# ahuang73/HemoCell

Hardware: AMD Instinct MI355X
Metric: MLUPS + cell-vertex updates/s, 256^3 pipeflow 10% Hct (higher is better)
Workload: dtype f64

## Files before the change

hemocell_amd/csrc/ibm.hip:

```cpp
#include "cells.h"
#include <hipcub/hipcub.hpp>
#include <cstdlib>
#include <cstring>
#include <numeric>

namespace {

__global__ __launch_bounds__(256) void ibm_spread_kernel(LatView v, long n, const double *px, const double *py, const double *pz,
                                                         double *fx, double *fy, double *fz, const double *rx, const double *ry, const double *rz,
                                                         double *F, int limit_on, double f_limit, const int *vert_cell, const int *tag, const unsigned char *dead) {
  const long i = (long)blockIdx.x * 256 + threadIdx.x;
  if (i >= n) return;
  if (dead[i] || tag[vert_cell[i]] == 1) return;
  double f0 = fx[i], f1 = fy[i], f2 = fz[i];
  if (limit_on) {
    const double mag = sqrt((f0 * f0 + f1 * f1) + f2 * f2);
    if (mag > f_limit) {
      const double sc = f_limit / mag;
      f0 *= sc; f1 *= sc; f2 *= sc;
      fx[i] = f0; fy[i] = f1; fz[i] = f2;
    }
  }
  Stencil s;
  phi2_stencil(v, px[i], py[i], pz[i], s);
#pragma unroll
  for (int k = 0; k < 8; k++) {
    if (s.node[k] < 0) continue;
    v.dirty[s.node[k] >> 4] = v.epoch;
    unsafeAtomicAdd(&F[s.node[k]], ((rx ? rx[i] : 0.0) + f0) * s.w[k]);
    unsafeAtomicAdd(&F[v.npad + s.node[k]], ((ry ? ry[i] : 0.0) + f1) * s.w[k]);
    unsafeAtomicAdd(&F[2 * v.npad + s.node[k]], ((rz ? rz[i] : 0.0) + f2) * s.w[k]);
  }
}

__global__ __launch_bounds__(256) void spread_emit_kernel(LatView v, int nv, long n, const int *order, long ebase, const double *px, const double *py,
                                                          const double *pz, double *fx, double *fy, double *fz, const double *rx, const double *ry,
                                                          const double *rz, int limit_on, double f_limit, const int *tag, const unsigned char *dead,
                                                          unsigned int *keys, int *vals, double *c0, double *c1, double *c2) {
  const long g = (long)blockIdx.x * 256 + threadIdx.x;
  if (g >= n) return;
  const int cell = order[g / nv];
  const long i = (long)cell * nv + (g % nv);
  const long e0 = (ebase + g) * 8;
  const bool live = tag[cell] != 1 && !dead[i];
  Stencil s;
  double f0 = 0.0, f1 = 0.0, f2 = 0.0;
  if (live) {
    f0 = fx[i]; f1 = fy[i]; f2 = fz[i];
    if (limit_on) {
      const double mag = sqrt((f0 * f0 + f1 * f1) + f2 * f2);
      if (mag > f_limit) { const double sc = f_limit / mag; f0 *= sc; f1 *= sc; f2 *= sc; fx[i] = f0; fy[i] = f1; fz[i] = f2; }
    }
    if (rx) { f0 = rx[i] + f0; f1 = ry[i] + f1; f2 = rz[i] + f2; }
    phi2_stencil(v, px[i], py[i], pz[i], s);
  }
#pragma unroll
  for (int k = 0; k < 8; k++) {
    const bool adm = live && s.node[k] >= 0;
    keys[e0 + k] = adm ? (unsigned int)s.node[k] : 0xffffffffu;
    vals[e0 + k] = (int)(e0 + k);
    c0[e0 + k] = adm ? f0 * s.w[k] : 0.0; c1[e0 + k] = adm ? f1 * s.w[k] : 0.0; c2[e0 + k] = adm ? f2 * s.w[k] : 0.0;
  }
}

__global__ __launch_bounds__(256) void spread_gather_kernel(LatView v, long n, const unsigned int *keys, const int *vals, const double *c0, const double *c1,
                                                            const double *c2, double *F) {
  const long s = (long)blockIdx.x * 256 + threadIdx.x;
  if (s >= n) return;
  const unsigned int key = keys[s];
  if (key == 0xffffffffu || (s > 0 && keys[s - 1] == key)) return;
  double a0 = 0.0, a1 = 0.0, a2 = 0.0;
  for (long q = s; q < n && keys[q] == key; q++) { const int e = vals[q]; a0 += c0[e]; a1 += c1[e]; a2 += c2[e]; }
  v.dirty[key >> 4] = v.epoch;
  F[key] += a0; F[v.npad + key] += a1; F[2 * v.npad + key] += a2;
}

struct PopView {
  const double *f; const double *F; double bx, by, bz; long qs;
  hc::BodyRegions reg;
};

__device__ __forceinline__ void node_velocity(const LatView &v, const PopView &pv, int lx, int ly, int lz, long node, double u[3]) {
  if (v.halo_x && (lx <= -HALO || lx >= v.nx + HALO - 1)) { u[0] = u[1] = u[2] = 0.0; return; }
  if (v.halo_x && (lx == -1 || lx == v.nx)) {
    const double *hu = v.halo_u[lx < 0 ? 0 : 1];
    if (hu) { const long k = (long)ly * v.nz + lz; u[0] = hu[k]; u[1] = hu[v.ny_nz + k]; u[2] = hu[2L * v.ny_nz + k]; return; }
  }
  long xm = -(long)v.plane, xp = (long)v.plane;
  if (v.wrap_x) { if (lx == 0) xm = (long)(v.nx - 1) * v.plane; if (lx == v.nx - 1) xp = -(long)(v.nx - 1) * v.plane; }
  int ym = -v.nz, yp = v.nz, zm = -1, zp = 1; bool ymk = true, ypk = true, zmk = true, zpk = true;
  if (ly == 0) { if (v.per_y) ym = (v.ny - 1) * v.nz; else ymk = false; }
  if (ly == v.ny - 1) { if (v.per_y) yp = -(v.ny - 1) * v.nz; else ypk = false; }
  if (lz == 0) { if (v.per_z) zm = v.nz - 1; else zmk = false; }
  if (lz == v.nz - 1) { if (v.per_z) zp = -(v.nz - 1); else zpk = false; }
  double r = 0.0, jx = 0.0, jy = 0.0, jz = 0.0;
#define M(Q, CX, CY, CZ)                                                              \
  {                                                                                   \
    long off = 0; bool ok = true;                                                     \
    if (CX == 1) off += xm; else if (CX == -1) off += xp;                             \
    if (CY == 1) { off += ym; ok = ok && ymk; } else if (CY == -1) { off += yp; ok = ok && ypk; } \
    if (CZ == 1) { off += zm; ok = ok && zmk; } else if (CZ == -1) { off += zp; ok = ok && zpk; } \
    const double fq = ok ? pv.f[(long)Q * pv.qs + node + off] : 0.0;                 \
    r += fq;                                                                          \
    if (CX == 1) jx += fq; else if (CX == -1) jx += -fq;                              \
    if (CY == 1) jy += fq; else if (CY == -1) jy += -fq;                              \
    if (CZ == 1) jz += fq; else if (CZ == -1) jz += -fq;                              \
  }
  M(0, 0, 0, 0) M(1, -1, 0, 0) M(2, 0, -1, 0) M(3, 0, 0, -1) M(4, -1, -1, 0) M(5, -1, 1, 0)
  M(6, -1, 0, -1) M(7, -1, 0, 1) M(8, 0, -1, -1) M(9, 0, -1, 1) M(10, 1, 0, 0) M(11, 0, 1, 0)
  M(12, 0, 0, 1) M(13, 1, 1, 0) M(14, 1, -1, 0) M(15, 1, 0, 1) M(16, 1, 0, -1) M(17, 0, 1, 1)
  M(18, 0, 1, -1)
#undef M
  const double invRho = 1.0 / (1.0 + r);
  double bx = pv.bx, by = pv.by, bz = pv.bz;
  if (pv.reg.n) {
    int xg = v.x0 + lx;
    if (xg < 0) xg += v.nx_global; else if (xg >= v.nx_global) xg -= v.nx_global;
    region_force(pv.reg, xg, ly, lz, bx, by, bz);
  }
  u[0] = jx * invRho + (bx + pv.F[node]) / 2.0;
  u[1] = jy * invRho + (by + pv.F[v.npad + node]) / 2.0;
  u[2] = jz * invRho + (bz + pv.F[2 * v.npad + node]) / 2.0;
}

__global__ __launch_bounds__(256) void face_velocity_kernel(LatView v, PopView pv, int lx0, double *out0, int lx1, double *out1) {
  const int k = blockIdx.x * 256 + threadIdx.x;
  if (k >= v.ny_nz) return;
  const int lx = blockIdx.y ? lx1 : lx0;
  double *out = blockIdx.y ? out1 : out0;
  const int ly = k / v.nz, lz = k - ly * v.nz;
  const long node = (long)(lx + HALO) * v.plane + (long)ly * v.nz + lz;
  double u[3] = {0.0, 0.0, 0.0};
  if (v.mask[node] == 0) node_velocity(v, pv, lx, ly, lz, node, u);
  out[k] = u[0]; out[v.ny_nz + k] = u[1]; out[2L * v.ny_nz + k] = u[2];
}

__global__ __launch_bounds__(256) void ibm_interpolate_kernel(LatView v, PopView pv, long n, const double *px, const double *py,
                                                              const double *pz, double *vx, double *vy, double *vz, const int *vert_cell, const int *tag,
                                                              const unsigned char *dead) {
  const long i = (long)blockIdx.x * 256 + threadIdx.x;
  if (i >= n) return;
  if (dead[i] || tag[vert_cell[i]] == 1) return;
  Stencil s;
  phi2_stencil(v, px[i], py[i], pz[i], s);
  double a0 = 0.0, a1 = 0.0, a2 = 0.0;
#pragma unroll
  for (int k = 0; k < 8; k++) {
    if (s.node[k] < 0) continue;
    double u[3];
    node_velocity(v, pv, s.lx[k], s.ly[k], s.lz[k], s.node[k], u);
    a0 += (u[0] * s.w[k]); a1 += (u[1] * s.w[k]); a2 += (u[2] * s.w[k]);
  }
  vx[i] = a0; vy[i] = a1; vz[i] = a2;
}


constexpr int TILE_CAP = 5832;
constexpr int NODE_CAP = 1536;

struct Tile { int o[3]; int e[3]; int vol; int ow[3]; float r1, r2; };

__device__ __forceinline__ void tile_decode(const Tile &t, int i, int &tx, int &ty, int &tz) {
  const int q = (int)(((float)i + 0.5f) * t.r2);
  tz = i - q * t.e[2];
  tx = (int)(((float)q + 0.5f) * t.r1);
  ty = q - tx * t.e[1];
}

__device__ __forceinline__ int stencil_base(const LatView &v, double px, double py, double pz, int b[3]) {
  const double p[3] = {px, py, pz};
#pragma unroll
  for (int a = 0; a < 3; a++) { const long c = nearest_node(p[a]); b[a] = (int)c + ((p[a] < (double)c) ? -1 : 0); }
  return 0;
}

// ... 110 lines not shown
  }
  if (!inside) return false;
  if (nb[0] * nb[1] * nb[2] > 64) return false;
  if (threadIdx.x < 64) {
    const int l = threadIdx.x;
    bool near = false;
    if (l < nb[0] * nb[1] * nb[2]) {
      const int bz = l % nb[2], by = (l / nb[2]) % nb[1], bx = l / (nb[2] * nb[1]);
      near = v.wallbrick[((long)(b0[0] + bx) * v.nby + (b0[1] + by)) * v.nbz + (b0[2] + bz)] != 0;
    }
    const unsigned long long any = __ballot(near);
    if (l == 0) *s_near = any != 0ull;
  }
  __syncthreads();
  return *s_near == 0;
}

__device__ __forceinline__ bool cell_prologue(const LatView &v, int nv, long base, const double *px, const double *py, const double *pz,
                                              const unsigned char *dead, int *s_red, int *s_near, unsigned char *mt, Tile &t, VStencil vs[NVPT] PH_PARAM) {
  const int tid = threadIdx.x, nth = blockDim.x;
  double p[NVPT][3]; int b[NVPT][3]; bool live[NVPT];
  int lo[3] = {0x7fffffff, 0x7fffffff, 0x7fffffff}, hi[3] = {-0x7fffffff, -0x7fffffff, -0x7fffffff};
#pragma unroll
  for (int j = 0; j < NVPT; j++) {
    const int i = tid + j * nth;
    live[j] = i < nv && !(dead && dead[base + i]);
    if (live[j]) {
      p[j][0] = px[base + i]; p[j][1] = py[base + i]; p[j][2] = pz[base + i];
      stencil_base(v, p[j][0], p[j][1], p[j][2], b[j]);
#pragma unroll
      for (int a = 0; a < 3; a++) { lo[a] = min(lo[a], b[j][a]); hi[a] = max(hi[a], b[j][a] + 1); }
    }
  }
  block_bbox(lo, hi, s_red, t);
  STAMP(1);
  if (!tile_finish(v, t) || nv > NVPT * nth) return false;
  const bool clear = tile_is_clear(v, t, s_near);
  STAMP(2);
  if (!clear) {
#pragma unroll 4
    for (int i = tid; i < t.vol; i += nth) mt[i] = tile_mask(v, t, i);
    __syncthreads();
  }
  STAMP(3);
#pragma unroll
  for (int j = 0; j < NVPT; j++) {
    vs[j].adm = 0; vs[j].base = 0;
    if (live[j]) tile_stencil(t, clear ? nullptr : mt, p[j][0], p[j][1], p[j][2], b[j], vs[j]);
  }
  STAMP(4);
  return true;
}

__global__ __launch_bounds__(256) void ibm_spread_cell_kernel(LatView v, int nv, const double *px, const double *py, const double *pz,
                                                              double *fx, double *fy, double *fz, const double *rx, const double *ry, const double *rz,
                                                              double *F, int limit_on, double f_limit, int xcd_ranges, const int *tag, const unsigned char *vdead) {
  __shared__ double tile[TILE_CAP];
  __shared__ unsigned char mt[TILE_CAP];
  __shared__ int s_red[6 * MAXW], s_near;
  const int tid = threadIdx.x, nth = blockDim.x;
  PH_INIT
  const int cell = xcd_ranges ? xcd_contiguous((int)blockIdx.x, (int)gridDim.x) : (int)blockIdx.x;
  const int state = tag[cell];
  if (state == 1) return;
  STAMP(0);
  const unsigned char *dead = state == 2 ? vdead : nullptr;
  const long base = (long)cell * nv;
  const bool in_regs = nv <= NVPT * nth;
  double f[NVPT][3];
  if (in_regs) {
#pragma unroll
    for (int j = 0; j < NVPT; j++) {
      const int i = tid + j * nth;
      f[j][0] = f[j][1] = f[j][2] = 0.0;
      if (i < nv) { f[j][0] = fx[base + i]; f[j][1] = fy[base + i]; f[j][2] = fz[base + i]; }
    }
  }
  Tile t; VStencil vs[NVPT];
  bool tiled = cell_prologue(v, nv, base, px, py, pz, dead, s_red, &s_near, mt, t, vs PH_ARG);
  if (limit_on) {
    if (in_regs) {
#pragma unroll
      for (int j = 0; j < NVPT; j++) {
        const int i = tid + j * nth;
        if (i < nv) {
          const double mag = sqrt((f[j][0] * f[j][0] + f[j][1] * f[j][1]) + f[j][2] * f[j][2]);
          if (mag > f_limit) { const double sc = f_limit / mag; f[j][0] *= sc; f[j][1] *= sc; f[j][2] *= sc; fx[base + i] = f[j][0]; fy[base + i] = f[j][1]; fz[base + i] = f[j][2]; }
        }
      }
    } else {
      for (int i = tid; i < nv; i += nth) {
        const double f0 = fx[base + i], f1 = fy[base + i], f2 = fz[base + i];
        const double mag = sqrt((f0 * f0 + f1 * f1) + f2 * f2);
        if (mag > f_limit) { const double sc = f_limit / mag; fx[base + i] = f0 * sc; fy[base + i] = f1 * sc; fz[base + i] = f2 * sc; }
      }
    }
  }
  if (!tiled) {
    for (int i = tid; i < nv; i += nth) {
      if (dead && dead[base + i]) continue;
      Stencil s;
      phi2_stencil(v, px[base + i], py[base + i], pz[base + i], s);
      const double f0 = (rx ? rx[base + i] : 0.0) + fx[base + i], f1 = (ry ? ry[base + i] : 0.0) + fy[base + i], f2 = (rz ? rz[base + i] : 0.0) + fz[base + i];
#pragma unroll
      for (int k = 0; k < 8; k++) {
        if (s.node[k] < 0) continue;
        v.dirty[s.node[k] >> 4] = v.epoch;
        unsafeAtomicAdd(&F[s.node[k]], f0 * s.w[k]);
        unsafeAtomicAdd(&F[v.npad + s.node[k]], f1 * s.w[k]);
        unsafeAtomicAdd(&F[2 * v.npad + s.node[k]], f2 * s.w[k]);
      }
    }
    return;
  }
  const int sy = t.e[2], sx = t.e[1] * t.e[2];
  for (int i = tid; i < t.vol; i += nth) tile[i] = 0.0;
  __syncthreads();
  STAMP(5);
#pragma unroll
  for (int comp = 0; comp < 3; comp++) {
    const double *rc = comp == 0 ? rx : comp == 1 ? ry : rz;
    double *Fc = F + (long)comp * v.npad;
#pragma unroll
    for (int j = 0; j < NVPT; j++) {
      const int i = tid + j * nth;
      if (i >= nv || !vs[j].adm) continue;
      const double fv = (rc ? rc[base + i] : 0.0) + f[j][comp];
#pragma unroll
      for (int k = 0; k < 8; k++)
        if (vs[j].adm & (1u << k)) atomicAdd(&tile[vs[j].base + (k >> 2) * sx + ((k >> 1) & 1) * sy + (k & 1)], fv * vs[j].w[k]);
    }
    __syncthreads();
    STAMP(6 + 2 * comp);
    for (int i = tid; i < t.vol; i += nth) {
      const double val = tile[i];
      if (val != 0.0) {
        if (comp < 2) tile[i] = 0.0;
        int lx, ly, lz; const long node = tile_node(v, t, i, lx, ly, lz); v.dirty[node >> 4] = v.epoch;
        unsafeAtomicAdd(&Fc[node], val);
      }
    }
    if (comp < 2) __syncthreads();
    STAMP(7 + 2 * comp);
  }
}

__global__ __launch_bounds__(256) void ibm_interpolate_cell_kernel(LatView v, PopView pv, int nv, const double *px, const double *py,
                                                                   const double *pz, double *vx, double *vy, double *vz, const int *slots, int xcd_ranges,
                                                                   const int *tag, const unsigned char *vdead) {
  constexpr unsigned short FREE = 0xFFFF, MARK = 0xFFFE;
  __shared__ unsigned short slot[TILE_CAP];
  __shared__ __attribute__((aligned(16))) unsigned char raw[TILE_CAP > 2 * NODE_CAP ? TILE_CAP : 2 * NODE_CAP];
  unsigned char *mt = raw; unsigned short *list = reinterpret_cast<unsigned short *>(raw);
  __shared__ double ux[NODE_CAP], uy[NODE_CAP], uz[NODE_CAP];
  __shared__ int s_red[6 * MAXW], s_count, s_near;
  const int tid = threadIdx.x, nth = blockDim.x;
  const int cell = slots ? slots[blockIdx.x] : (xcd_ranges ? xcd_contiguous((int)blockIdx.x, (int)gridDim.x) : (int)blockIdx.x);
  const int state = tag[cell];
  if (state == 1) return;
  const unsigned char *dead = state == 2 ? vdead : nullptr;
  const long base = (long)cell * nv;
  Tile t; VStencil vs[NVPT];
  PH_INIT
  bool tiled = cell_prologue(v, nv, base, px, py, pz, dead, s_red, &s_near, mt, t, vs PH_ARG);
  const int sy = t.e[2], sx = t.e[1] * t.e[2];
  if (tiled) {
    for (int i = tid; i < t.vol; i += nth) slot[i] = FREE;
    if (tid == 0) s_count = 0;
    __syncthreads();
#pragma unroll
    for (int j = 0; j < NVPT; j++)
#pragma unroll
      for (int k = 0; k < 8; k++) if (vs[j].adm & (1u << k)) slot[vs[j].base + (k >> 2) * sx + ((k >> 1) & 1) * sy + (k & 1)] = MARK;
    __syncthreads();
    for (int i0 = 0; i0 < t.vol; i0 += nth) {
      const int i = i0 + tid;
      const bool marked = i < t.vol && slot[i] == MARK;
      const unsigned long long b = __ballot(marked);
      int first = 0;
      if ((tid & 63) == 0 && b) first = atomicAdd(&s_count, (int)__popcll(b));
      first = __shfl(first, 0);
      if (marked) {
        const int n = first + (int)__popcll(b & ((1ull << (tid & 63)) - 1ull));
        if (n < NODE_CAP) { slot[i] = (unsigned short)n; list[n] = (unsigned short)i; }
      }
    }
    __syncthreads();
    STAMP(12);
    if (s_count > NODE_CAP) tiled = false;
  }
  if (tiled) {
    const int n = s_count;
    for (int k = tid; k < n; k += nth) {
      int lx, ly, lz;
      const long node = tile_node(v, t, list[k], lx, ly, lz);
      double u[3];
      node_velocity(v, pv, lx, ly, lz, node, u);
      ux[k] = u[0]; uy[k] = u[1]; uz[k] = u[2];
    }
    __syncthreads();
    STAMP(13);
#pragma unroll
    for (int j = 0; j < NVPT; j++) {
      const int i = tid + j * nth;
      if (i >= nv) continue;
      double a0 = 0.0, a1 = 0.0, a2 = 0.0;
#pragma unroll
      for (int k = 0; k < 8; k++) {
        if (!(vs[j].adm & (1u << k))) continue;
        const int q = slot[vs[j].base + (k >> 2) * sx + ((k >> 1) & 1) * sy + (k & 1)];
        a0 += (ux[q] * vs[j].w[k]); a1 += (uy[q] * vs[j].w[k]); a2 += (uz[q] * vs[j].w[k]);
      }
      vx[base + i] = a0; vy[base + i] = a1; vz[base + i] = a2;
    }
    STAMP(14);
    return;
  }
  for (int i = tid; i < nv; i += nth) {
    if (dead && dead[base + i]) continue;
    Stencil s;
    phi2_stencil(v, px[base + i], py[base + i], pz[base + i], s);
    double a0 = 0.0, a1 = 0.0, a2 = 0.0;
#pragma unroll
    for (int k = 0; k < 8; k++) {
      if (s.node[k] < 0) continue;
      double u[3];
      node_velocity(v, pv, s.lx[k], s.ly[k], s.lz[k], s.node[k], u);
      a0 += (u[0] * s.w[k]); a1 += (u[1] * s.w[k]); a2 += (u[2] * s.w[k]);
    }
    vx[base + i] = a0; vy[base + i] = a1; vz[base + i] = a2;
  }
}

}

static int g_ibm_per_vertex = 0;
extern "C" int hc_debug_ibm_per_vertex(int on) { g_ibm_per_vertex = on; return HC_OK; }
static int g_reproducible = -1;
static bool reproducible() {
  if (g_reproducible < 0) { const char *e = std::getenv("HEMOCELL_REPRODUCIBLE_SPREAD"); g_reproducible = (e && *e && *e != '0') ? 1 : 0; }
  return g_reproducible == 1;
}
// ... 180 lines not shown
```

hemocell_amd/csrc/lattice.hip:

```cpp
#include "common.h"
#include "comm.h"
#include <algorithm>

using namespace hc;

namespace {

struct LatArgs {
  const double *fin;
  double *fout;
  const double *Fin;
  double *Fzero;
  const uint8_t *mask;
  int nx, ny, nz;
  int plane;
  long xs;
  long npad;
  long qs;
  int x_begin;
  int x_split, x_jump;
  int wrap_x, per_y, per_z;
  double omega;
  double bx, by, bz;
  const int *row_z0, *row_cum, *blk_row;
// ... 87 lines not shown
  if (CZ != 0) { double t = (CZ == 1 ? a2 : -a2); s = first ? t : s + t; first = false; }
  return s;
}

__device__ __forceinline__ void collide_guo(double f[HC_Q], double Fx, double Fy, double Fz, double omega) {
  double rhoBar, j0, j1, j2;
  moments(f, rhoBar, j0, j1, j2);
  const double invRho = 1.0 / (1.0 + rhoBar);
  const double rho = 1.0 + rhoBar;
  const double u0 = j0 * invRho + Fx / 2.0, u1 = j1 * invRho + Fy / 2.0, u2 = j2 * invRho + Fz / 2.0;
  j0 = rho * u0; j1 = rho * u1; j2 = rho * u2;
  const double jSqr = j0 * j0 + j1 * j1 + j2 * j2;
  const double one_m_omega = 1.0 - omega;
  const double guo = 1.0 - omega / 2.0;
#define M(Q, CX, CY, CZ)                                                                     \
  {                                                                                          \
    const double c_j = cdot<CX, CY, CZ>(j0, j1, j2);                                         \
    const double feq = tq(Q) * (rhoBar + 3.0 * c_j + invRho * (4.5 * c_j * c_j - 1.5 * jSqr)); \
    f[Q] *= one_m_omega;                                                                     \
    f[Q] += omega * feq;                                                                     \
  }
  FOR_Q(M)
#undef M
#define M(Q, CX, CY, CZ)                                                                     \
  {                                                                                          \
    double c_u = cdot<CX, CY, CZ>(u0, u1, u2);                                               \
    c_u *= 9.0;                                                                              \
    double ft = (((double)CX - u0) * 3.0 + c_u * (double)CX) * Fx;                           \
    ft += (((double)CY - u1) * 3.0 + c_u * (double)CY) * Fy;                                 \
    ft += (((double)CZ - u2) * 3.0 + c_u * (double)CZ) * Fz;                                 \
    ft *= tq(Q);                                                                             \
    ft *= guo;                                                                               \
    f[Q] += ft;                                                                              \
  }
  FOR_Q(M)
#undef M
}

template <bool REGIONS>
__global__ __launch_bounds__(256) void collide_stream_kernel(LatArgs a) {
  const int x = a.x_begin + (int)blockIdx.y + ((int)blockIdx.y >= a.x_split ? a.x_jump : 0);
  const int xp = x + HALO;
  const int t = blockIdx.x * 256 + threadIdx.x;
  const int *cum = a.row_cum + (long)xp * (a.ny + 1);
  if (t >= cum[a.ny]) return;
  int lo = a.blk_row[(long)xp * (a.nblk + 1) + blockIdx.x], hi = a.blk_row[(long)xp * (a.nblk + 1) + blockIdx.x + 1];
  while (lo < hi) { const int mid = (lo + hi + 1) >> 1; if (cum[mid] <= t) lo = mid; else hi = mid - 1; }
  const int y = lo, z = a.row_z0[(long)xp * a.ny + y] + (t - cum[y]);
  const int p = y * a.nz + z;
  const long node = (long)(x + HALO) * a.xs + p;
  const uint8_t m = a.mask[node];
  if (m == 2) return;
  const Nbr n = neighbours(a, x, y, z);
  double f[HC_Q];
  pull(a.fin, a.qs, node, n, f);
  const bool wall = m != 0;
  if (wall) {
#pragma unroll
    for (int i = 1; i <= 9; i++) { double t = f[i]; f[i] = f[i + 9]; f[i + 9] = t; }
    if (m >= 3) {
      const double w0 = a.wall_u[m - 3][0], w1 = a.wall_u[m - 3][1], w2 = a.wall_u[m - 3][2];
#define M(Q, CX, CY, CZ)                                                                  \
      if (Q != 0) {                                                                       \
        constexpr int O = Q <= 9 ? Q + 9 : Q - 9;                                         \
        const double c_u = (double)CX * w0 + (double)CY * w1 + (double)CZ * w2;           \
        f[O] = f[O] - 6.0 * tq(Q) * c_u;                                                  \
      }
      FOR_Q(M)
#undef M
    }
  } else {
    double bx = a.bx, by = a.by, bz = a.bz;
    if (REGIONS) region_force(a.reg, a.x0 + x, y, z, bx, by, bz);
    double Fx = bx, Fy = by, Fz = bz;
    if (a.ibm && a.dirty_in[node >> 4] == a.epoch_in) {
      Fx = bx + a.Fin[node]; Fy = by + a.Fin[a.npad + node]; Fz = bz + a.Fin[2 * a.npad + node];
    }
    collide_guo(f, Fx, Fy, Fz, a.omega);
  }
#pragma unroll
  for (int q = 0; q < HC_Q; q++) __builtin_nontemporal_store(f[q], &a.fout[(long)q * a.qs + node]);
  if (a.ibm && a.dirty_zero[node >> 4] == a.epoch_zero) { a.Fzero[node] = 0.0; a.Fzero[a.npad + node] = 0.0; a.Fzero[2 * a.npad + node] = 0.0; }
}

__global__ void init_eq_kernel(LatArgs a, double rhoBar, double j0, double j1, double j2) {
  const int p = blockIdx.x * 256 + threadIdx.x;
  if (p >= a.plane) return;
  const int x = a.x_begin + blockIdx.y;
  const int y = p / a.nz, z = p - y * a.nz;
  const long node = (long)(x + HALO) * a.xs + p;
  const Nbr n = neighbours(a, x, y, z);
  const double invRho = 1.0 / (1.0 + rhoBar);
  const double jSqr = j0 * j0 + j1 * j1 + j2 * j2;
#define M(Q, CX, CY, CZ)                                                                        \
  {                                                                                             \
    bool ok; long off = dst_off<CX, CY, CZ>(n, ok);                                             \
    double v = 0.0;                                                                             \
    if (ok && a.mask[node + off] == 0) {                                                        \
      const double c_j = cdot<CX, CY, CZ>(j0, j1, j2);                                          \
      v = tq(Q) * (rhoBar + 3.0 * c_j + invRho * (4.5 * c_j * c_j - 1.5 * jSqr));               \
    }                                                                                           \
    a.fout[(long)Q * a.qs + node] = v;                                                          \
  }
  FOR_Q(M)
#undef M
}

__global__ void download_kernel(LatArgs a, double *aos) {
  const int p = blockIdx.x * 256 + threadIdx.x;
  if (p >= a.plane) return;
  const int x = a.x_begin + blockIdx.y;
  const int y = p / a.nz, z = p - y * a.nz;
  const long node = (long)(x + HALO) * a.xs + p;
  const Nbr n = neighbours(a, x, y, z);
  double f[HC_Q];
  pull(a.fin, a.qs, node, n, f);
  const long o = ((long)x * a.plane + p) * HC_Q;
#pragma unroll
  for (int q = 0; q < HC_Q; q++) aos[o + q] = f[q];
}

__global__ void upload_kernel(LatArgs a, const double *aos, int lo_ok, int hi_ok) {
  const int p = blockIdx.x * 256 + threadIdx.x;
  if (p >= a.plane) return;
  const int x = a.x_begin + blockIdx.y;
  const int y = p / a.nz, z = p - y * a.nz;
  const long node = (long)(x + HALO) * a.xs + p;
  const long bulk = (long)x * a.plane + p;
  Nbr nl = neighbours(a, x, y, z);
  nl.xm = nl.xm / a.xs * a.plane; nl.xp = nl.xp / a.xs * a.plane;
#define M(Q, CX, CY, CZ)                                                                  \
  {                                                                                       \
    bool ok; long off = dst_off<CX, CY, CZ>(nl, ok);                                      \
     \
    if (!a.wrap_x && ((CX == 1 && x == a.nx - 1 && !hi_ok) || (CX == -1 && x == 0 && !lo_ok))) ok = false; \
    a.fout[(long)Q * a.qs + node] = ok ? aos[(bulk + off) * HC_Q + Q] : 0.0;            \
  }
  FOR_Q(M)
#undef M
}

__global__ void rho_u_kernel(LatArgs a, double *rho, double *u) {
  const int p = blockIdx.x * 256 + threadIdx.x;
  if (p >= a.plane) return;
  const int x = a.x_begin + blockIdx.y;
  const int y = p / a.nz, z = p - y * a.nz;
  const long node = (long)(x + HALO) * a.xs + p;
  const Nbr n = neighbours(a, x, y, z);
  double f[HC_Q];
  pull(a.fin, a.qs, node, n, f);
  double rhoBar, j0, j1, j2;
  moments(f, rhoBar, j0, j1, j2);
  const double invRho = 1.0 / (1.0 + rhoBar);
  const long o = (long)x * a.plane + p;
  rho[o] = 1.0 + rhoBar;
  double bx, by, bz;
  body_at(a, x, y, z, bx, by, bz);
  u[3 * o] = j0 * invRho + (bx + a.Fin[node]) / 2.0;
  u[3 * o + 1] = j1 * invRho + (by + a.Fin[a.npad + node]) / 2.0;
  u[3 * o + 2] = j2 * invRho + (bz + a.Fin[2 * a.npad + node]) / 2.0;
}

__global__ void pi_neq_kernel(LatArgs a, double *pi) {
  const int p = blockIdx.x * 256 + threadIdx.x;
  if (p >= a.plane) return;
  const int x = a.x_begin + blockIdx.y;
  const int y = p / a.nz, z = p - y * a.nz;
  const long node = (long)(x + HALO) * a.xs + p;
  const Nbr n = neighbours(a, x, y, z);
  double f[HC_Q];
  pull(a.fin, a.qs, node, n, f);
  double rhoBar, j0, j1, j2;
  moments(f, rhoBar, j0, j1, j2);
  const double invRho = 1.0 / (1.0 + rhoBar);
  double xx = 0, xy = 0, xz = 0, yy = 0, yz = 0, zz = 0;
#define M(Q, CX, CY, CZ)                       \
  if (CX * CX) xx += f[Q];                     \
  if (CX * CY == 1) xy += f[Q]; else if (CX * CY == -1) xy += -f[Q]; \
  if (CX * CZ == 1) xz += f[Q]; else if (CX * CZ == -1) xz += -f[Q]; \
  if (CY * CY) yy += f[Q];                     \
  if (CY * CZ == 1) yz += f[Q]; else if (CY * CZ == -1) yz += -f[Q]; \
  if (CZ * CZ) zz += f[Q];
  FOR_Q(M)
#undef M
  const double cs2 = 1.0 / 3.0;
  const long o = 6 * ((long)x * a.plane + p);
  pi[o] = xx - invRho * j0 * j0 - cs2 * rhoBar;
  pi[o + 1] = xy - invRho * j0 * j1;
  pi[o + 2] = xz - invRho * j0 * j2;
  pi[o + 3] = yy - invRho * j1 * j1 - cs2 * rhoBar;
  pi[o + 4] = yz - invRho * j1 * j2;
  pi[o + 5] = zz - invRho * j2 * j2 - cs2 * rhoBar;
}

__global__ void force_aos_kernel(LatArgs a, double *F) {
  const int p = blockIdx.x * 256 + threadIdx.x;
  if (p >= a.plane) return;
  const int x = a.x_begin + blockIdx.y;
  const long node = (long)(x + HALO) * a.xs + p;
  const long o = (long)x * a.plane + p;
  for (int d = 0; d < 3; d++) F[3 * o + d] = a.Fin[d * a.npad + node];
}

__global__ __launch_bounds__(256) void fluid_stats_kernel(LatArgs a, int what, double *partial) {
  StatAcc acc{1e300, -1e300, 0.0, 0};
  const long nbulk = (long)a.nx * a.plane;
  for (long k = (long)blockIdx.x * 256 + threadIdx.x; k < nbulk; k += (long)STAT_BLOCKS * 256) {
    const int x = (int)(k / a.plane), p = (int)(k - (long)x * a.plane);
    const long node = (long)(x + HALO) * a.xs + p;
    if (what == 2) {
      double r = 0.0;
#pragma unroll
      for (int q = 0; q < HC_Q; q++) r += a.fin[(long)q * a.qs + node];
      stat_add(acc, r);
      continue;
    }
    if (a.mask[node] != 0) continue;
    const int y = p / a.nz, z = p - y * a.nz;
    double bx, by, bz;
    body_at(a, x, y, z, bx, by, bz);
    double Fx = bx, Fy = by, Fz = bz;
    if (a.ibm) { Fx = bx + a.Fin[node]; Fy = by + a.Fin[a.npad + node]; Fz = bz + a.Fin[2 * a.npad + node]; }
    double v0 = Fx, v1 = Fy, v2 = Fz;
    if (what == 0) {
      const Nbr n = neighbours(a, x, y, z);
      double f[HC_Q];
      pull(a.fin, a.qs, node, n, f);
      double rhoBar, j0, j1, j2;
      moments(f, rhoBar, j0, j1, j2);
      const double invRho = 1.0 / (1.0 + rhoBar);
      v0 = j0 * invRho + Fx / 2.0; v1 = j1 * invRho + Fy / 2.0; v2 = j2 * invRho + Fz / 2.0;
    }
    stat_add(acc, sqrt(v0 * v0 + v1 * v1 + v2 * v2));
  }
  stat_block_store(acc, partial);
}


__device__ __forceinline__ void collide_external(double f[HC_Q], double rhoBar, double j0, double j1, double j2, double omega) {
  const double invRho = 1.0 / (1.0 + rhoBar);
  const double jSqr = j0 * j0 + j1 * j1 + j2 * j2;
  const double one_m_omega = 1.0 - omega;
#define M(Q, CX, CY, CZ)                                                                     \
  {                                                                                          \
    const double c_j = cdot<CX, CY, CZ>(j0, j1, j2);                                         \
    const double feq = tq(Q) * (rhoBar + 3.0 * c_j + invRho * (4.5 * c_j * c_j - 1.5 * jSqr)); \
    f[Q] *= one_m_omega;                                                                     \
    f[Q] += omega * feq;                                                                     \
  }
  FOR_Q(M)
#undef M
}

__device__ __forceinline__ long modp(long a, long b) { return (a % b + b) % b; }

__global__ __launch_bounds__(256) void le_gather_kernel(LatArgs a, double *buf, double D, double v_top, double v_bottom) {
  const long nxy = (long)a.nx * a.ny;
  const long t = (long)blockIdx.x * 256 + threadIdx.x;
  if (t >= 2 * nxy) return;
  const int top = t < nxy ? 1 : 0;
  const long r = top ? t : t - nxy;
  const int x = (int)(r / a.ny), y = (int)(r - (long)x * a.ny);
  const int z = top ? a.nz - 1 : 0;
  const long row = (long)y * a.nz + z;
  const long node = (long)(x + HALO) * a.xs + row;
  double f[HC_Q];
  pull(a.fin, a.qs, node, neighbours(a, x, y, z), f);
  double rhoBar = 0.0;
#pragma unroll
  for (int q = 0; q < HC_Q; q++) rhoBar += f[q];
  collide_external(f, rhoBar, top ? v_top : v_bottom, 0.0, 0.0, a.omega);
  const double g = fmod(D, 1.0);
  const long s1 = top ? modp((long)ceil(D + (double)x), a.nx) : modp((long)floor(-D + (double)x), a.nx);
  const long s2 = top ? modp((long)floor(D + (double)x), a.nx) : modp((long)ceil(-D + (double)x), a.nx);
  double f1[HC_Q], f2[HC_Q];
// ... 6 lines not shown
    f[16] = g * f1[6] + (1 - g) * f2[6];
    f[18] = g * f1[18] + (1 - g) * f2[18];
  } else {
    f[7] = g * f1[15] + (1 - g) * f2[15];
    f[9] = g * f1[9] + (1 - g) * f2[9];
    f[12] = g * f1[12] + (1 - g) * f2[12];
    f[15] = g * f1[7] + (1 - g) * f2[7];
    f[17] = g * f1[17] + (1 - g) * f2[17];
  }
  double *o = buf + (long)(1 - top) * HC_Q * nxy + r;
#pragma unroll
  for (int q = 0; q < HC_Q; q++) o[(long)q * nxy] = f[q];
}

__global__ __launch_bounds__(256) void le_scatter_kernel(LatArgs a, const double *buf) {
  const long nxy = (long)a.nx * a.ny;
  const long t = (long)blockIdx.x * 256 + threadIdx.x;
  if (t >= 2 * nxy) return;
  const int top = t < nxy ? 1 : 0;
  const long r = top ? t : t - nxy;
  const int x = (int)(r / a.ny), y = (int)(r - (long)x * a.ny);
  const int z = top ? a.nz - 1 : 0;
  const long node = (long)(x + HALO) * a.xs + (long)y * a.nz + z;
  const Nbr n = neighbours(a, x, y, z);
  const double *in = buf + (long)(1 - top) * HC_Q * nxy + r;
#define M(Q, CX, CY, CZ)                                                       \
  {                                                                            \
    bool ok; const long off = src_off<CX, CY, CZ>(n, ok);                      \
    if (ok) a.fout[(long)Q * a.qs + node + off] = in[(long)Q * nxy];           \
  }
  FOR_Q(M)
#undef M
}

struct HaloArgs {
  double *f;
  double *buf;
  double *buf2; int n_first;
  long npad; long xs; int plane;
  int n;
  int pop[HC_Q + 5];
  int xp[HC_Q + 5];
  int to_buf;
};
__global__ void halo_copy_kernel(HaloArgs h) {
  const int p = blockIdx.x * 256 + threadIdx.x;
  if (p >= h.plane) return;
  const int e = blockIdx.y;
  const long li = (long)h.pop[e] * h.npad + (long)h.xp[e] * h.xs + p;
  double *b = e < h.n_first ? h.buf + (long)e * h.plane + p : h.buf2 + (long)(e - h.n_first) * h.plane + p;
  if (h.to_buf) *b = h.f[li]; else h.f[li] = *b;
}

__global__ void zero_force_halo_kernel(double *F, long npad, long xs, int plane, int nx) {
  const int p = blockIdx.x * 256 + threadIdx.x;
  if (p >= plane) return;
  const int comp = blockIdx.y / (2 * HALO), w = blockIdx.y % (2 * HALO);
  const int xp = w < HALO ? w : nx + w;
  F[(long)comp * npad + (long)xp * xs + p] = 0.0;
}

LatArgs make_args(const hc_lattice *L) {
  LatArgs a;
  a.fin = L->f[L->cur]; a.fout = L->f[1 - L->cur];
  const int fprev = (L->fcur + 2) % 3;
  a.Fin = L->force[L->fcur]; a.Fzero = L->force[fprev];
  a.x_split = 0x7fffffff; a.x_jump = 0;
  a.mask = L->mask;
  a.nx = L->nx; a.ny = L->ny; a.nz = L->nz; a.plane = (int)L->plane; a.xs = (long)L->xs; a.npad = (long)L->npad; a.qs = (long)L->qstride;
  a.x_begin = 0;
  a.wrap_x = (L->n_slabs == 1 && L->periodic[0]) ? 1 : 0;
  a.per_y = L->periodic[1]; a.per_z = L->periodic[2];
  a.omega = L->omega; a.bx = L->body[0]; a.by = L->body[1]; a.bz = L->body[2];
  a.x0 = L->x0; a.nx_global = L->nx_global; a.reg = L->regions;
  a.row_z0 = L->row_z0; a.row_cum = L->row_cum; a.blk_row = L->blk_row; a.nblk = L->nblk;
  a.ibm = L->ibm;
  a.dirty_in = L->fdirty[L->fcur]; a.dirty_zero = L->fdirty[fprev]; a.epoch_in = L->fepoch[L->fcur]; a.epoch_zero = L->fepoch[fprev];
  for (int c = 0; c < 4; c++) for (int d = 0; d < 3; d++) a.wall_u[c][d] = L->wall_u[c][d];
  return a;
}

dim3 plane_grid(const hc_lattice *L, int nplanes) { return dim3((unsigned)((L->plane + 255) / 256), (unsigned)nplanes, 1); }

int ensure_scratch(hc_lattice *L, size_t doubles) {
  if (L->scratch_doubles >= doubles) return HC_OK;
  if (L->scratch) HC_HIP(hipFree(L->scratch));
  L->scratch = nullptr; L->scratch_doubles = 0;
  HC_HIP(hipMalloc((void **)&L->scratch, doubles * sizeof(double)));
  L->scratch_doubles = doubles;
  return HC_OK;
}

int rebuild_active_map(hc_lattice *L) {
  const int NX = L->nx + 2 * HALO, ny = L->ny, nz = L->nz;
  std::vector<int> z0((size_t)NX * ny), cum((size_t)NX * (ny + 1));
  int max_active = 0;
  for (int x = 0; x < NX; x++) {
    int c = 0;
    for (int y = 0; y < ny; y++) {
      const uint8_t *row = L->hmask.data() + (size_t)x * L->xs + (size_t)y * nz;
      int a = 0, b = nz;
      while (a < nz && row[a] == 2) a++;
      while (b > a && row[b - 1] == 2) b--;
      z0[(size_t)x * ny + y] = a;
      cum[(size_t)x * (ny + 1) + y] = c;
      c += b - a;
    }
    cum[(size_t)x * (ny + 1) + ny] = c;
    max_active = std::max(max_active, c);
  }
  if (max_active == 0) max_active = 1;
  const int nblk = (max_active + 255) / 256;
// ... 222 lines not shown
  LatArgs a = make_args(L);
  a.fout = L->f[L->cur];
  HC_HIP(hipMemsetAsync(L->f[0], 0, L->qstride * HC_Q * sizeof(double), hc::stream()));
  HC_HIP(hipMemsetAsync(L->f[1], 0, L->qstride * HC_Q * sizeof(double), hc::stream()));
  hipLaunchKernelGGL(init_eq_kernel, plane_grid(L, L->nx), dim3(256), 0, hc::stream(), a, rho - 1.0, rho * u[0], rho * u[1], rho * u[2]);
  HC_HIP(hipGetLastError());
  HC_HIP(hipStreamSynchronize(hc::stream()));
  return HC_OK;
}

int hcl_set_wall_velocity(hc_lattice *L, int wall_class, const double u[3]) {
  HC_REQUIRE(L && u && wall_class >= 3 && wall_class <= 6, "hcl_set_wall_velocity: class must be 3..6");
  for (int d = 0; d < 3; d++) L->wall_u[wall_class - 3][d] = u[d];
  return HC_OK;
}

int hcl_set_body_force(hc_lattice *L, const double F[3]) {
  HC_REQUIRE(L && F, "hcl_set_body_force: null pointer");
  for (int d = 0; d < 3; d++) L->body[d] = F[d];
  return HC_OK;
}

int hcl_set_body_force_regions(hc_lattice *L, int n, const int *boxes, const double *forces) {
  HC_REQUIRE(L && n >= 0 && (n == 0 || (boxes && forces)), "hcl_set_body_force_regions: bad arguments");
  HC_REQUIRE(n <= HC_MAX_FORCE_REGIONS, "hcl_set_body_force_regions: more than HC_MAX_FORCE_REGIONS boxes");
  for (int k = 0; k < n; k++) {
    const int *b = boxes + 6 * k;
    HC_REQUIRE(b[0] <= b[1] && b[2] <= b[3] && b[4] <= b[5], "hcl_set_body_force_regions: empty box");
    for (int i = 0; i < 6; i++) L->regions.box[k][i] = b[i];
    for (int d = 0; d < 3; d++) L->regions.f[k][d] = forces[3 * k + d];
  }
  L->regions.n = n;
  return HC_OK;
}

int hcl_collide_stream_part(hc_lattice *L, int part) {
  HC_REQUIRE(L, "hcl_collide_stream_part: null lattice");
  HC_REQUIRE(part >= 0 && part <= 6, "hcl_collide_stream_part: part must be 0..6");
  HC_REQUIRE(part < 3 || L->nx >= 4, "hcl_collide_stream_part: parts 3, 4 and 6 need a slab of at least 4 planes");
  hc::ProfScope prof(hc::forked() ? hc::PK_COLLIDE_BESIDE : hc::PK_COLLIDE);
  int rc = HC_OK;
  if (part == 0) rc = launch_collide(L, 0, L->nx);
  else if (part == 1) rc = launch_collide(L, 1, L->nx - 2);
  else if (part == 2 || part == 5) rc = launch_collide(L, 0, 1, L->nx - 1, 1);
  else if (part == 3) rc = launch_collide(L, 2, L->nx - 4);
  else rc = launch_collide(L, 0, 2, L->nx - 2, 2);
  if (rc == HC_OK && (part == 0 || part == 2 || part == 4)) rc = hcl_zero_force_halos(L);
  return rc;
}

int hcl_zero_force_halos(hc_lattice *L) {
  HC_REQUIRE(L, "hcl_zero_force_halos: null lattice");
  if (L->n_slabs <= 1 || !L->ibm) return HC_OK;
  hipLaunchKernelGGL(zero_force_halo_kernel, dim3((unsigned)((L->plane + 255) / 256), (unsigned)(2 * HALO * 3), 1), dim3(256), 0, hc::stream(),
                     L->force[(L->fcur + 2) % 3], (long)L->npad, (long)L->xs, (int)L->plane, L->nx);
  HC_HIP(hipGetLastError());
  return HC_OK;
}

int hcl_step_end(hc_lattice *L) {
  HC_REQUIRE(L, "hcl_step_end: null lattice");
  L->cur ^= 1; L->fcur = (L->fcur + 1) % 3;
  L->halo_u_valid = false;
  L->fepoch[L->fcur] = (uint8_t)(L->fepoch[L->fcur] % 255 + 1);
  return HC_OK;
}

int hcl_collide_stream(hc_lattice *L, int nsteps) {
  HC_REQUIRE(L, "hcl_collide_stream: null lattice");
  if (L->n_slabs > 1) return hcs::collide_stream_slab(L, nsteps);
  for (int s = 0; s < nsteps; s++) {
    int rc = hcl_collide_stream_part(L, 0);
    if (rc != HC_OK) return rc;
    hcl_step_end(L);
    if ((rc = hc::lees_edwards_step(L)) != HC_OK) return rc;
  }
  return HC_OK;
}

int hcl_set_lees_edwards(hc_lattice *L, double v_top, double v_bottom) {
  HC_REQUIRE(L, "hcl_set_lees_edwards: null lattice");
  HC_REQUIRE(L->n_slabs == 1, "hcl_set_lees_edwards: the Lees-Edwards boundary needs the whole domain on one GPU (n_slabs = 1)");
  HC_REQUIRE(L->periodic[0] && L->periodic[1] && L->periodic[2], "hcl_set_lees_edwards: the lattice must be periodic on all three axes");
  HC_REQUIRE(L->nz >= 4, "hcl_set_lees_edwards: nz must be at least 4");
  if (!le_layers_fluid(L, L->hmask.data(), L->xs)) {
    hc::set_error("hcl_set_lees_edwards: the layers z = 0, 1, nz-2 and nz-1 must hold fluid nodes only");
    return HC_ERR_STATE;
  }
  if (!L->le_buf) HC_HIP(hipMalloc((void **)&L->le_buf, (size_t)2 * HC_Q * L->nx * L->ny * sizeof(double)));
  L->le_on = true; L->le_v_top = v_top; L->le_v_bottom = v_bottom; L->le_D = 0.0; L->le_d = 0.0;
  return HC_OK;
}

int hcl_set_lees_edwards_displacement(hc_lattice *L, double D, double d_per_iteration) {
  HC_REQUIRE(L, "hcl_set_lees_edwards_displacement: null lattice");
  if (!L->le_on) { hc::set_error("hcl_set_lees_edwards_displacement: no Lees-Edwards boundary (hcl_set_lees_edwards)"); return HC_ERR_STATE; }
  L->le_D = D; L->le_d = d_per_iteration;
  return HC_OK;
}

int hcl_lees_edwards_apply(hc_lattice *L) {
  HC_REQUIRE(L, "hcl_lees_edwards_apply: null lattice");
  if (!L->le_on) { hc::set_error("hcl_lees_edwards_apply: no Lees-Edwards boundary (hcl_set_lees_edwards)"); return HC_ERR_STATE; }
  return launch_lees_edwards(L);
}

int hcl_lees_edwards_state(const hc_lattice *L, double out[4]) {
  HC_REQUIRE(L && out, "hcl_lees_edwards_state: null pointer");
// ... 159 lines not shown
```

Baseline: 15170.

## Interleave IBM force field as AoS and compact spread accumulation per touched node

Switches the force field from three component planes (SoA) to interleaved xyz per node. The collide kernel, interpolation, spread and halo zeroing all index it as F[3*node+d], so one node's three components share a cache line. The per-cell spread kernel now compacts the touched tile nodes into a dense list and accumulates all three components in one pass of shared-memory atomics. This replaces three full-tile passes with per-component syncs, and it falls back to direct global atomics when the node count exceeds capacity. The risk is a strided rather than coalesced force read in the collide kernel, and any unconverted force consumer or halo code that still assumes the planar layout.

```diff
diff --git a/hemocell_amd/csrc/ibm.hip b/hemocell_amd/csrc/ibm.hip
--- a/hemocell_amd/csrc/ibm.hip
+++ b/hemocell_amd/csrc/ibm.hip
@@ -27,9 +27,10 @@
   for (int k = 0; k < 8; k++) {
     if (s.node[k] < 0) continue;
     v.dirty[s.node[k] >> 4] = v.epoch;
-    unsafeAtomicAdd(&F[s.node[k]], ((rx ? rx[i] : 0.0) + f0) * s.w[k]);
-    unsafeAtomicAdd(&F[v.npad + s.node[k]], ((ry ? ry[i] : 0.0) + f1) * s.w[k]);
-    unsafeAtomicAdd(&F[2 * v.npad + s.node[k]], ((rz ? rz[i] : 0.0) + f2) * s.w[k]);
+    double *Fn = F + 3 * s.node[k];
+    unsafeAtomicAdd(Fn, ((rx ? rx[i] : 0.0) + f0) * s.w[k]);
+    unsafeAtomicAdd(Fn + 1, ((ry ? ry[i] : 0.0) + f1) * s.w[k]);
+    unsafeAtomicAdd(Fn + 2, ((rz ? rz[i] : 0.0) + f2) * s.w[k]);
   }
 }
 
@@ -72,7 +73,8 @@
   double a0 = 0.0, a1 = 0.0, a2 = 0.0;
   for (long q = s; q < n && keys[q] == key; q++) { const int e = vals[q]; a0 += c0[e]; a1 += c1[e]; a2 += c2[e]; }
   v.dirty[key >> 4] = v.epoch;
-  F[key] += a0; F[v.npad + key] += a1; F[2 * v.npad + key] += a2;
+  double *Fn = F + 3 * (long)key;
+  Fn[0] += a0; Fn[1] += a1; Fn[2] += a2;
 }
 
 struct PopView {
@@ -118,9 +120,9 @@
     if (xg < 0) xg += v.nx_global; else if (xg >= v.nx_global) xg -= v.nx_global;
     region_force(pv.reg, xg, ly, lz, bx, by, bz);
   }
-  u[0] = jx * invRho + (bx + pv.F[node]) / 2.0;
-  u[1] = jy * invRho + (by + pv.F[v.npad + node]) / 2.0;
-  u[2] = jz * invRho + (bz + pv.F[2 * v.npad + node]) / 2.0;
+  u[0] = jx * invRho + (bx + pv.F[3 * node]) / 2.0;
+  u[1] = jy * invRho + (by + pv.F[3 * node + 1]) / 2.0;
+  u[2] = jz * invRho + (bz + pv.F[3 * node + 2]) / 2.0;
 }
 
 __global__ __launch_bounds__(256) void face_velocity_kernel(LatView v, PopView pv, int lx0, double *out0, int lx1, double *out1) {
@@ -337,12 +339,62 @@
   return true;
 }
 
+constexpr unsigned short SLOT_FREE = 0xFFFF, SLOT_MARK = 0xFFFE;
+__device__ __forceinline__ int compact_nodes(const Tile &t, const VStencil vs[NVPT], unsigned short *slot, unsigned short *list, int *s_count) {
+  const int tid = threadIdx.x, nth = blockDim.x;
+  const int sy = t.e[2], sx = t.e[1] * t.e[2];
+  for (int i = tid; i < t.vol; i += nth) slot[i] = SLOT_FREE;
+  if (tid == 0) *s_count = 0;
+  __syncthreads();
+#pragma unroll
+  for (int j = 0; j < NVPT; j++)
+#pragma unroll
+    for (int k = 0; k < 8; k++) if (vs[j].adm & (1u << k)) slot[vs[j].base + (k >> 2) * sx + ((k >> 1) & 1) * sy + (k & 1)] = SLOT_MARK;
+  __syncthreads();
+  for (int i0 = 0; i0 < t.vol; i0 += nth) {
+    const int i = i0 + tid;
+    const bool marked = i < t.vol && slot[i] == SLOT_MARK;
+    const unsigned long long b = __ballot(marked);
+    int first = 0;
+    if ((tid & 63) == 0 && b) first = atomicAdd(s_count, (int)__popcll(b));
+    first = __shfl(first, 0);
+    if (marked) {
+      const int n = first + (int)__popcll(b & ((1ull << (tid & 63)) - 1ull));
+      if (n < NODE_CAP) { slot[i] = (unsigned short)n; list[n] = (unsigned short)i; }
+    }
+  }
+  __syncthreads();
+  return *s_count;
+}
+
+__device__ void spread_direct(const LatView &v, int nv, long base, const double *px, const double *py, const double *pz, const double *fx,
+                              const double *fy, const double *fz, const double *rx, const double *ry, const double *rz, double *F,
+                              const unsigned char *dead) {
+  for (int i = threadIdx.x; i < nv; i += blockDim.x) {
+    if (dead && dead[base + i]) continue;
+    Stencil s;
+    phi2_stencil(v, px[base + i], py[base + i], pz[base + i], s);
+    const double f0 = (rx ? rx[base + i] : 0.0) + fx[base + i], f1 = (ry ? ry[base + i] : 0.0) + fy[base + i], f2 = (rz ? rz[base + i] : 0.0) + fz[base + i];
+#pragma unroll
+    for (int k = 0; k < 8; k++) {
+      if (s.node[k] < 0) continue;
+      v.dirty[s.node[k] >> 4] = v.epoch;
+      double *Fn = F + 3 * s.node[k];
+      unsafeAtomicAdd(Fn, f0 * s.w[k]);
+      unsafeAtomicAdd(Fn + 1, f1 * s.w[k]);
+      unsafeAtomicAdd(Fn + 2, f2 * s.w[k]);
+    }
+  }
+}
+
 __global__ __launch_bounds__(256) void ibm_spread_cell_kernel(LatView v, int nv, const double *px, const double *py, const double *pz,
                                                               double *fx, double *fy, double *fz, const double *rx, const double *ry, const double *rz,
                                                               double *F, int limit_on, double f_limit, int xcd_ranges, const int *tag, const unsigned char *vdead) {
-  __shared__ double tile[TILE_CAP];
-  __shared__ unsigned char mt[TILE_CAP];
-  __shared__ int s_red[6 * MAXW], s_near;
+  __shared__ unsigned short slot[TILE_CAP];
+  __shared__ __attribute__((aligned(16))) unsigned char raw[TILE_CAP > 2 * NODE_CAP ? TILE_CAP : 2 * NODE_CAP];
+  unsigned char *mt = raw; unsigned short *list = reinterpret_cast<unsigned short *>(raw);
+  __shared__ double acc[3 * NODE_CAP];
+  __shared__ int s_red[6 * MAXW], s_count, s_near;
   const int tid = threadIdx.x, nth = blockDim.x;
   PH_INIT
   const int cell = xcd_ranges ? xcd_contiguous((int)blockIdx.x, (int)gridDim.x) : (int)blockIdx.x;
@@ -381,59 +433,41 @@
       }
     }
   }
-  if (!tiled) {
-    for (int i = tid; i < nv; i += nth) {
-      if (dead && dead[base + i]) continue;
-      Stencil s;
-      phi2_stencil(v, px[base + i], py[base + i], pz[base + i], s);
-      const double f0 = (rx ? rx[base + i] : 0.0) + fx[base + i], f1 = (ry ? ry[base + i] : 0.0) + fy[base + i], f2 = (rz ? rz[base + i] : 0.0) + fz[base + i];
-#pragma unroll
-      for (int k = 0; k < 8; k++) {
-        if (s.node[k] < 0) continue;
-        v.dirty[s.node[k] >> 4] = v.epoch;
-        unsafeAtomicAdd(&F[s.node[k]], f0 * s.w[k]);
-        unsafeAtomicAdd(&F[v.npad + s.node[k]], f1 * s.w[k]);
-        unsafeAtomicAdd(&F[2 * v.npad + s.node[k]], f2 * s.w[k]);
-      }
-    }
-    return;
-  }
+  const int n = tiled ? compact_nodes(t, vs, slot, list, &s_count) : 0;
+  STAMP(5);
+  if (!tiled || n > NODE_CAP) { spread_direct(v, nv, base, px, py, pz, fx, fy, fz, rx, ry, rz, F, dead); return; }
   const int sy = t.e[2], sx = t.e[1] * t.e[2];
-  for (int i = tid; i < t.vol; i += nth) tile[i] = 0.0;
+  for (int k = tid; k < 3 * n; k += nth) acc[k] = 0.0;
   __syncthreads();
-  STAMP(5);
-#pragma unroll
-  for (int comp = 0; comp < 3; comp++) {
-    const double *rc = comp == 0 ? rx : comp == 1 ? ry : rz;
-    double *Fc = F + (long)comp * v.npad;
-#pragma unroll
-    for (int j = 0; j < NVPT; j++) {
-      const int i = tid + j * nth;
-      if (i >= nv || !vs[j].adm) continue;
-      const double fv = (rc ? rc[base + i] : 0.0) + f[j][comp];
-#pragma unroll
-      for (int k = 0; k < 8; k++)
-        if (vs[j].adm & (1u << k)) atomicAdd(&tile[vs[j].base + (k >> 2) * sx + ((k >> 1) & 1) * sy + (k & 1)], fv * vs[j].w[k]);
-    }
-    __syncthreads();
-    STAMP(6 + 2 * comp);
-    for (int i = tid; i < t.vol; i += nth) {
-      const double val = tile[i];
-      if (val != 0.0) {
-        if (comp < 2) tile[i] = 0.0;
-        int lx, ly, lz; const long node = tile_node(v, t, i, lx, ly, lz); v.dirty[node >> 4] = v.epoch;
-        unsafeAtomicAdd(&Fc[node], val);
-      }
-    }
-    if (comp < 2) __syncthreads();
-    STAMP(7 + 2 * comp);
-  }
+#pragma unroll
+  for (int j = 0; j < NVPT; j++) {
+    const int i = tid + j * nth;
+    if (i >= nv || !vs[j].adm) continue;
+    double fv[3];
+    fv[0] = (rx ? rx[base + i] : 0.0) + f[j][0]; fv[1] = (ry ? ry[base + i] : 0.0) + f[j][1]; fv[2] = (rz ? rz[base + i] : 0.0) + f[j][2];
+#pragma unroll
+    for (int k = 0; k < 8; k++) {
+      if (!(vs[j].adm & (1u << k))) continue;
+      double *a = &acc[3 * slot[vs[j].base + (k >> 2) * sx + ((k >> 1) & 1) * sy + (k & 1)]];
+      atomicAdd(a, fv[0] * vs[j].w[k]); atomicAdd(a + 1, fv[1] * vs[j].w[k]); atomicAdd(a + 2, fv[2] * vs[j].w[k]);
+    }
+  }
+  __syncthreads();
+  STAMP(6);
+  for (int k = tid; k < 3 * n; k += nth) {
+    const double val = acc[k];
+    if (val != 0.0) {
+      const int q = k / 3;
+      int lx, ly, lz; const long node = tile_node(v, t, list[q], lx, ly, lz); v.dirty[node >> 4] = v.epoch;
+      unsafeAtomicAdd(&F[3 * node + (k - 3 * q)], val);
+    }
+  }
+  STAMP(7);
 }
 
 __global__ __launch_bounds__(256) void ibm_interpolate_cell_kernel(LatView v, PopView pv, int nv, const double *px, const double *py,
                                                                    const double *pz, double *vx, double *vy, double *vz, const int *slots, int xcd_ranges,
                                                                    const int *tag, const unsigned char *vdead) {
-  constexpr unsigned short FREE = 0xFFFF, MARK = 0xFFFE;
   __shared__ unsigned short slot[TILE_CAP];
   __shared__ __attribute__((aligned(16))) unsigned char raw[TILE_CAP > 2 * NODE_CAP ? TILE_CAP : 2 * NODE_CAP];
   unsigned char *mt = raw; unsigned short *list = reinterpret_cast<unsigned short *>(raw);
@@ -450,29 +484,8 @@
   bool tiled = cell_prologue(v, nv, base, px, py, pz, dead, s_red, &s_near, mt, t, vs PH_ARG);
   const int sy = t.e[2], sx = t.e[1] * t.e[2];
   if (tiled) {
-    for (int i = tid; i < t.vol; i += nth) slot[i] = FREE;
-    if (tid == 0) s_count = 0;
-    __syncthreads();
-#pragma unroll
-    for (int j = 0; j < NVPT; j++)
-#pragma unroll
-      for (int k = 0; k < 8; k++) if (vs[j].adm & (1u << k)) slot[vs[j].base + (k >> 2) * sx + ((k >> 1) & 1) * sy + (k & 1)] = MARK;
-    __syncthreads();
-    for (int i0 = 0; i0 < t.vol; i0 += nth) {
-      const int i = i0 + tid;
-      const bool marked = i < t.vol && slot[i] == MARK;
-      const unsigned long long b = __ballot(marked);
-      int first = 0;
-      if ((tid & 63) == 0 && b) first = atomicAdd(&s_count, (int)__popcll(b));
-      first = __shfl(first, 0);
-      if (marked) {
-        const int n = first + (int)__popcll(b & ((1ull << (tid & 63)) - 1ull));
-        if (n < NODE_CAP) { slot[i] = (unsigned short)n; list[n] = (unsigned short)i; }
-      }
-    }
-    __syncthreads();
+    if (compact_nodes(t, vs, slot, list, &s_count) > NODE_CAP) tiled = false;
     STAMP(12);
-    if (s_count > NODE_CAP) tiled = false;
   }
   if (tiled) {
     const int n = s_count;
diff --git a/hemocell_amd/csrc/lattice.hip b/hemocell_amd/csrc/lattice.hip
--- a/hemocell_amd/csrc/lattice.hip
+++ b/hemocell_amd/csrc/lattice.hip
@@ -163,6 +163,9 @@
   const uint8_t m = a.mask[node];
   if (m == 2) return;
   const Nbr n = neighbours(a, x, y, z);
+  const bool fdirty = a.ibm && m == 0 && a.dirty_in[node >> 4] == a.epoch_in;
+  double F0 = 0.0, F1 = 0.0, F2 = 0.0;
+  if (fdirty) { F0 = a.Fin[3 * node]; F1 = a.Fin[3 * node + 1]; F2 = a.Fin[3 * node + 2]; }
   double f[HC_Q];
   pull(a.fin, a.qs, node, n, f);
   const bool wall = m != 0;
@@ -184,14 +187,14 @@
     double bx = a.bx, by = a.by, bz = a.bz;
     if (REGIONS) region_force(a.reg, a.x0 + x, y, z, bx, by, bz);
     double Fx = bx, Fy = by, Fz = bz;
-    if (a.ibm && a.dirty_in[node >> 4] == a.epoch_in) {
-      Fx = bx + a.Fin[node]; Fy = by + a.Fin[a.npad + node]; Fz = bz + a.Fin[2 * a.npad + node];
+    if (fdirty) {
+      Fx = bx + F0; Fy = by + F1; Fz = bz + F2;
     }
     collide_guo(f, Fx, Fy, Fz, a.omega);
   }
 #pragma unroll
   for (int q = 0; q < HC_Q; q++) __builtin_nontemporal_store(f[q], &a.fout[(long)q * a.qs + node]);
-  if (a.ibm && a.dirty_zero[node >> 4] == a.epoch_zero) { a.Fzero[node] = 0.0; a.Fzero[a.npad + node] = 0.0; a.Fzero[2 * a.npad + node] = 0.0; }
+  if (a.ibm && a.dirty_zero[node >> 4] == a.epoch_zero) { a.Fzero[3 * node] = 0.0; a.Fzero[3 * node + 1] = 0.0; a.Fzero[3 * node + 2] = 0.0; }
 }
 
 __global__ void init_eq_kernel(LatArgs a, double rhoBar, double j0, double j1, double j2) {
@@ -267,9 +270,9 @@
   rho[o] = 1.0 + rhoBar;
   double bx, by, bz;
   body_at(a, x, y, z, bx, by, bz);
-  u[3 * o] = j0 * invRho + (bx + a.Fin[node]) / 2.0;
-  u[3 * o + 1] = j1 * invRho + (by + a.Fin[a.npad + node]) / 2.0;
-  u[3 * o + 2] = j2 * invRho + (bz + a.Fin[2 * a.npad + node]) / 2.0;
+  u[3 * o] = j0 * invRho + (bx + a.Fin[3 * node]) / 2.0;
+  u[3 * o + 1] = j1 * invRho + (by + a.Fin[3 * node + 1]) / 2.0;
+  u[3 * o + 2] = j2 * invRho + (bz + a.Fin[3 * node + 2]) / 2.0;
 }
 
 __global__ void pi_neq_kernel(LatArgs a, double *pi) {
@@ -310,7 +313,7 @@
   const int x = a.x_begin + blockIdx.y;
   const long node = (long)(x + HALO) * a.xs + p;
   const long o = (long)x * a.plane + p;
-  for (int d = 0; d < 3; d++) F[3 * o + d] = a.Fin[d * a.npad + node];
+  for (int d = 0; d < 3; d++) F[3 * o + d] = a.Fin[3 * node + d];
 }
 
 __global__ __launch_bounds__(256) void fluid_stats_kernel(LatArgs a, int what, double *partial) {
@@ -331,7 +334,7 @@
     double bx, by, bz;
     body_at(a, x, y, z, bx, by, bz);
     double Fx = bx, Fy = by, Fz = bz;
-    if (a.ibm) { Fx = bx + a.Fin[node]; Fy = by + a.Fin[a.npad + node]; Fz = bz + a.Fin[2 * a.npad + node]; }
+    if (a.ibm) { Fx = bx + a.Fin[3 * node]; Fy = by + a.Fin[3 * node + 1]; Fz = bz + a.Fin[3 * node + 2]; }
     double v0 = Fx, v1 = Fy, v2 = Fz;
     if (what == 0) {
       const Nbr n = neighbours(a, x, y, z);
@@ -444,12 +447,12 @@
   if (h.to_buf) *b = h.f[li]; else h.f[li] = *b;
 }
 
-__global__ void zero_force_halo_kernel(double *F, long npad, long xs, int plane, int nx) {
-  const int p = blockIdx.x * 256 + threadIdx.x;
-  if (p >= plane) return;
-  const int comp = blockIdx.y / (2 * HALO), w = blockIdx.y % (2 * HALO);
+__global__ void zero_force_halo_kernel(double *F, long xs, int plane, int nx) {
+  const int e = blockIdx.x * 256 + threadIdx.x;
+  if (e >= 3 * plane) return;
+  const int w = blockIdx.y;
   const int xp = w < HALO ? w : nx + w;
-  F[(long)comp * npad + (long)xp * xs + p] = 0.0;
+  F[3 * (long)xp * xs + e] = 0.0;
 }
 
 LatArgs make_args(const hc_lattice *L) {
@@ -778,8 +781,8 @@
 int hcl_zero_force_halos(hc_lattice *L) {
   HC_REQUIRE(L, "hcl_zero_force_halos: null lattice");
   if (L->n_slabs <= 1 || !L->ibm) return HC_OK;
-  hipLaunchKernelGGL(zero_force_halo_kernel, dim3((unsigned)((L->plane + 255) / 256), (unsigned)(2 * HALO * 3), 1), dim3(256), 0, hc::stream(),
-                     L->force[(L->fcur + 2) % 3], (long)L->npad, (long)L->xs, (int)L->plane, L->nx);
+  hipLaunchKernelGGL(zero_force_halo_kernel, dim3((unsigned)((3 * L->plane + 255) / 256), (unsigned)(2 * HALO), 1), dim3(256), 0, hc::stream(),
+                     L->force[(L->fcur + 2) % 3], (long)L->xs, (int)L->plane, L->nx);
   HC_HIP(hipGetLastError());
   return HC_OK;
 }
```

After: 15740, median of 6. +3.8%, better.
